# zkMIPS/zkm

Hardware: AMD Instinct MI355X
Metric: segment_proofs_per_sec (higher is better)
Workload: dtype u64 (Goldilocks p = 2^64 - 2^32 + 1, integer modular)

## Files before the change

include/zkm_hip.h:

```cpp
#ifndef ZKM_HIP_H
#define ZKM_HIP_H
#include <stddef.h>
#include <stdint.h>
#ifdef __cplusplus
extern "C" {
#endif

typedef struct zkm_ctx zkm_ctx;
typedef struct zkm_batch zkm_batch;

int zkm_ctx_create(int device, zkm_ctx** out, char** err);
void zkm_ctx_destroy(zkm_ctx* ctx);
int zkm_ctx_synchronize(zkm_ctx* ctx, char** err);
uint64_t zkm_ctx_host_waits(const zkm_ctx* ctx);
void* zkm_ctx_stream(zkm_ctx* ctx);
void zkm_ctx_memory(const zkm_ctx* ctx, size_t* live_bytes, size_t* cached_bytes);
size_t zkm_ctx_resident_bytes(const zkm_ctx* ctx);
void zkm_ctx_trim(zkm_ctx* ctx);
int zkm_ctx_set_tuning(zkm_ctx* ctx, const char* key, uint64_t value, char** err);
int zkm_host_alloc(zkm_ctx* ctx, size_t bytes, void** out, char** err);
int zkm_host_free(zkm_ctx* ctx, void* p);
int zkm_host_register(zkm_ctx* ctx, void* p, size_t bytes, char** err);
int zkm_host_unregister(zkm_ctx* ctx, void* p);
int zkm_dev_alloc(zkm_ctx* ctx, size_t bytes, void** out, char** err);
// ... 30 lines not shown
#define ZKM_POSEIDON_PROBE_PERMUTE_LANE_MFMA 1
#define ZKM_POSEIDON_PROBE_PERMUTE_QUAD 2
#define ZKM_POSEIDON_PROBE_PERMUTE_WIDE 3
#define ZKM_POSEIDON_PROBE_MDS_VALU 4
#define ZKM_POSEIDON_PROBE_MDS_MFMA 5
#define ZKM_POSEIDON_PROBE_MDS_QUAD 6
#define ZKM_POSEIDON_PROBE_MDS_ROWS 7
#define ZKM_POSEIDON_PROBE_GROUP3 8
#define ZKM_POSEIDON_PROBE_GROUP3_QUAD 9
#define ZKM_POSEIDON_PROBE_GROUP2 10
#define ZKM_POSEIDON_PROBE_FOLD 11
#define ZKM_POSEIDON_PROBE_FOLD_TY 12
#define ZKM_POSEIDON_PROBE_SBOX7 13
#define ZKM_POSEIDON_PROBE_SBOX_DELTA 14
#define ZKM_POSEIDON_PROBE_ADD_RC0 15
int zkm_poseidon_selftest(zkm_ctx* ctx, uint32_t probe, uint32_t arg, const uint64_t* in, size_t n, uint64_t* out, char** err);

int zkm_consumer_selftest(zkm_ctx* ctx, const uint64_t* alphas, size_t nalphas, const uint64_t* terms, size_t K, size_t n, uint32_t run,
                          uint64_t* out, char** err);

#define ZKM_POSEIDON_COLS 262
int zkm_poseidon_trace(zkm_ctx* ctx, uint64_t seed, size_t num_perms, unsigned log_n, uint64_t* out_dev, char** err);

int zkm_poseidon_trace_inputs(zkm_ctx* ctx, const uint64_t* inputs, const uint64_t* timestamps, size_t num_perms, unsigned log_n,
                              uint64_t* out_dev, char** err);

#define ZKM_POSEIDON_SPONGE_COLS 110
int zkm_poseidon_sponge_trace(zkm_ctx* ctx, const uint8_t* inputs, const uint64_t* input_off, const uint64_t* meta, size_t nops,
                              unsigned log_n, uint64_t* out_dev, size_t* rows_used_out, char** err);

// ... 483 lines not shown
```

integration/rust/zkm_hip_sys.rs:

```rust
#![allow(non_camel_case_types)]
use std::os::raw::{c_char, c_double, c_int, c_uint, c_void};

#[repr(C)] pub struct zkm_ctx { _p: [u8; 0] }
#[repr(C)] pub struct zkm_batch { _p: [u8; 0] }
#[repr(C)] pub struct zkm_pool { _p: [u8; 0] }
#[repr(C)] pub struct zkm_staged { _p: [u8; 0] }
pub enum zkm_staged_ops {}

#[repr(C)] #[derive(Clone, Copy, Debug, Default)]
pub struct zkm_challenger { pub state: [u64; 12], pub in_buf: [u64; 8], pub out_buf: [u64; 8], pub n_in: u32, pub n_out: u32 }

#[repr(C)] #[derive(Clone, Copy, Debug)]
pub struct zkm_stark_config { pub rate_bits: c_uint, pub cap_height: c_uint, pub pow_bits: c_uint, pub num_challenges: c_uint,
                              pub num_queries: c_uint, pub arity_bits: c_uint, pub final_poly_bits: c_uint }

#[repr(C)] #[derive(Clone, Copy, Debug, Default)]
pub struct zkm_proof_layout {
    pub degree_bits: u64, pub trace_cols: u64, pub aux_cols: u64, pub quotient_polys: u64, pub ctl_zs: u64, pub cap_height: u64,
    pub fri_layers: u64, pub final_poly_len: u64, pub num_queries: u64, pub rate_bits: u64, pub arity_bits: u64,
    pub total_words: usize, pub init_challenger_state: usize, pub trace_cap: usize, pub aux_cap: usize, pub quotient_cap: usize,
    pub local_values: usize, pub next_values: usize, pub aux_polys: usize, pub aux_polys_next: usize, pub ctl_zs_first: usize,
    pub quotient_polys_open: usize, pub commit_phase_merkle_caps: usize, pub final_poly: usize, pub pow_witness: usize,
    pub query_round_proofs: usize, pub query_round_words: usize,
}
// ... 114 lines not shown
pub const ZKM_INSN_LUI: u32 = 0; pub const ZKM_INSN_MUL: u32 = 1; pub const ZKM_INSN_MULT: u32 = 2; pub const ZKM_INSN_MULTU: u32 = 3;
pub const ZKM_INSN_DIV: u32 = 4; pub const ZKM_INSN_DIVU: u32 = 5; pub const ZKM_INSN_MFHI: u32 = 6; pub const ZKM_INSN_MTHI: u32 = 7;
pub const ZKM_INSN_MFLO: u32 = 8; pub const ZKM_INSN_MTLO: u32 = 9; pub const ZKM_INSN_SDC1: u32 = 10; pub const ZKM_INSN_SYNC: u32 = 11;
pub const ZKM_INSN_PREF: u32 = 12;
pub const ZKM_VERIFY_OK: u32 = 0; pub const ZKM_VERIFY_SHAPE: u32 = 1; pub const ZKM_VERIFY_TRANSCRIPT_STATE: u32 = 2;
pub const ZKM_VERIFY_CTL_CHALLENGES: u32 = 3; pub const ZKM_VERIFY_QUOTIENT: u32 = 4; pub const ZKM_VERIFY_POW: u32 = 5;
pub const ZKM_VERIFY_INITIAL_MERKLE: u32 = 6; pub const ZKM_VERIFY_FRI_EVAL: u32 = 7; pub const ZKM_VERIFY_FRI_MERKLE: u32 = 8;
pub const ZKM_VERIFY_FINAL_POLY: u32 = 9; pub const ZKM_VERIFY_CTL_SUM: u32 = 10; pub const ZKM_VERIFY_FAILED: u32 = 11;

pub const ZKM_POSEIDON_OUT_ALL: u32 = 0; pub const ZKM_POSEIDON_OUT_CAPACITY: u32 = 1; pub const ZKM_POSEIDON_OUT_DIGEST: u32 = 2;
pub const ZKM_POSEIDON_PROBE_PERMUTE_LANE: u32 = 0; pub const ZKM_POSEIDON_PROBE_PERMUTE_LANE_MFMA: u32 = 1; pub const ZKM_POSEIDON_PROBE_PERMUTE_QUAD: u32 = 2;
pub const ZKM_POSEIDON_PROBE_PERMUTE_WIDE: u32 = 3; pub const ZKM_POSEIDON_PROBE_MDS_VALU: u32 = 4; pub const ZKM_POSEIDON_PROBE_MDS_MFMA: u32 = 5;
pub const ZKM_POSEIDON_PROBE_MDS_QUAD: u32 = 6; pub const ZKM_POSEIDON_PROBE_MDS_ROWS: u32 = 7; pub const ZKM_POSEIDON_PROBE_GROUP3: u32 = 8;
pub const ZKM_POSEIDON_PROBE_GROUP3_QUAD: u32 = 9; pub const ZKM_POSEIDON_PROBE_GROUP2: u32 = 10; pub const ZKM_POSEIDON_PROBE_FOLD: u32 = 11;
pub const ZKM_POSEIDON_PROBE_FOLD_TY: u32 = 12; pub const ZKM_POSEIDON_PROBE_SBOX7: u32 = 13; pub const ZKM_POSEIDON_PROBE_SBOX_DELTA: u32 = 14;
pub const ZKM_POSEIDON_PROBE_ADD_RC0: u32 = 15;
pub const ZKM_TABLE_POSEIDON: c_int = 0; pub const ZKM_TABLE_LOGIC: c_int = 1; pub const ZKM_TABLE_KECCAK_SPONGE: c_int = 2;
pub const ZKM_TABLE_KECCAK: c_int = 3; pub const ZKM_TABLE_MEMORY: c_int = 4; pub const ZKM_TABLE_POSEIDON_SPONGE: c_int = 5;
pub const ZKM_TABLE_SHA_EXTEND: c_int = 6; pub const ZKM_TABLE_SHA_EXTEND_SPONGE: c_int = 7; pub const ZKM_TABLE_SHA_COMPRESS: c_int = 8;
pub const ZKM_TABLE_SHA_COMPRESS_SPONGE: c_int = 9; pub const ZKM_TABLE_ARITHMETIC: c_int = 10; pub const ZKM_TABLE_CPU: c_int = 11;
pub const ZKM_MEMORY_COLS: usize = 13;
pub const ZKM_ARITHMETIC_COLS: usize = 54;

#[link(name = "zkmhip")]
extern "C" {
    pub fn zkm_ctx_create(device: c_int, out: *mut *mut zkm_ctx, err: *mut *mut c_char) -> c_int;
    pub fn zkm_ctx_destroy(ctx: *mut zkm_ctx);
    pub fn zkm_ctx_synchronize(ctx: *mut zkm_ctx, err: *mut *mut c_char) -> c_int;
    pub fn zkm_ctx_stream(ctx: *mut zkm_ctx) -> *mut c_void;
    pub fn zkm_ctx_memory(ctx: *const zkm_ctx, live_bytes: *mut usize, cached_bytes: *mut usize);
    pub fn zkm_ctx_resident_bytes(ctx: *const zkm_ctx) -> usize;
// ... 288 lines not shown
```

zkm_amd/__init__.py:

```python
import ctypes as C
import os
import re
import subprocess
import weakref

import numpy as np

_HERE = os.path.dirname(os.path.abspath(__file__))
_CSRC = os.path.join(_HERE, "csrc")
_LIB_PATH = os.environ.get("ZKM_HIP_LIB") or os.path.join(_CSRC, "libzkmhip.so")

P = 0xFFFFFFFF00000001


class ZkmError(RuntimeError):
    pass


from . import abi

_H = abi.constants("ZKM_")
POSEIDON_COLS, KECCAK_SPONGE_COLS, LOGIC_COLS, MEMORY_COLS, ARITHMETIC_COLS, KECCAK_COLS, POSEIDON_SPONGE_COLS = (
    _H[n + "_COLS"] for n in ("POSEIDON", "KECCAK_SPONGE", "LOGIC", "MEMORY", "ARITHMETIC", "KECCAK", "POSEIDON_SPONGE"))
TABLE_POSEIDON, TABLE_LOGIC, TABLE_KECCAK_SPONGE, TABLE_KECCAK, TABLE_MEMORY, TABLE_POSEIDON_SPONGE = 0, 1, 2, 3, 4, 5
# ... 923 lines not shown
    def ntt(self, cols, ncols, log_n, inverse=False, coset_shift=0):
        err = C.c_char_p()
        _check(self.L.zkm_ntt(self.h, _data_ptr(cols), ncols, log_n, int(inverse), coset_shift, C.byref(err)), err)
        return cols

    def field_selftest(self, a, b):
        a, b = np.ascontiguousarray(a, dtype=np.uint64), np.ascontiguousarray(b, dtype=np.uint64)
        out = np.zeros(7 * a.size, dtype=np.uint64)
        err = C.c_char_p()
        _check(self.L.zkm_field_selftest(self.h, a.ctypes.data_as(u64p), b.ctypes.data_as(u64p), a.size, out.ctypes.data_as(u64p), C.byref(err)), err)
        return out.reshape(7, -1)

    def poseidon_selftest(self, probe, arg, words):
        probe = POSEIDON_PROBE[probe] if isinstance(probe, str) else int(probe)
        words = np.ascontiguousarray(words, dtype=np.uint64).reshape(-1)
        pairs = probe in (POSEIDON_PROBE["FOLD"], POSEIDON_PROBE["FOLD_TY"])
        per = 2 if pairs else 12
        if words.size % per:
            raise ValueError("poseidon_selftest: %d words are not a whole number of %s" % (words.size, "pairs" if pairs else "states"))
        n = words.size // per
        out = np.zeros(n if pairs else 12 * n, dtype=np.uint64)
        err = C.c_char_p()
        _check(self.L.zkm_poseidon_selftest(self.h, probe, int(arg), words.ctypes.data_as(u64p), n, out.ctypes.data_as(u64p), C.byref(err)), err)
        return out if pairs else out.reshape(-1, 12)

    def consumer_selftest(self, alphas, terms, run=8):
        alphas = np.ascontiguousarray(alphas, dtype=np.uint64).reshape(-1)
        terms = np.ascontiguousarray(terms, dtype=np.uint64)
        if terms.ndim != 2:
            raise ValueError("consumer_selftest: terms must be a (K, n) array")
        K, n = terms.shape
        out = np.zeros(alphas.size * n, dtype=np.uint64)
        err = C.c_char_p()
        _check(self.L.zkm_consumer_selftest(self.h, alphas.ctypes.data_as(u64p), alphas.size, terms.ctypes.data_as(u64p), K, n, int(run),
# ... 1158 lines not shown
```

zkm_amd/csrc/hash.hip:

```cpp
#include <atomic>
#include "poseidon_dev.h"
#include "poseidon_lat_dev.h"
#include "poseidon_mfma_dev.h"
#include "hash_constants_dev.h"
#include "zkm_internal.h"

#ifndef ZKM_LEAF_MFMA_WAVES
#define ZKM_LEAF_MFMA_WAVES (ZKM_MFMA_PARK ? 5 : 4)
#endif

#ifndef ZKM_LATENCY_PRIO
#define ZKM_LATENCY_PRIO 3
#endif
#define ZKM_RAISE_PRIO()                                              \
    do {                                                              \
        if (ZKM_LATENCY_PRIO) __builtin_amdgcn_s_setprio(ZKM_LATENCY_PRIO); \
    } while (0)

__global__ __launch_bounds__(256) void k_poseidon_permute(gl_t* states, size_t k) {
    size_t i = (size_t)blockIdx.x * blockDim.x + threadIdx.x;
    if (i >= k) return;
    uint64_t s[12];
#pragma unroll
    for (int j = 0; j < 12; j++) s[j] = states[i * 12 + j];
// ... 200 lines not shown
                f.template load<true>(s, src, c, nw);
                sponge_lane_valu().permute(s, POSEIDON_OUT_ALL);
            }
        }
    }
    if constexpr (CHUNK) {
        if (!last) {
            f.store_state(s, state, n);
            return;
        }
    }
    f.store_digest(s, digests, f.item, f.live);
}

#define ZKM_LEAF_MFMA_ATTR __attribute__((amdgpu_waves_per_eu(ZKM_LEAF_MFMA_WAVES, ZKM_LEAF_MFMA_WAVES)))

__global__ __launch_bounds__(256) void k_merkle_leaves(const gl_t* __restrict__ lde, size_t nrows, size_t ncols, size_t col_stride,
                                                       gl_t* __restrict__ digests, size_t lde_seg, size_t dig_seg) {
    merkle_leaves_body<sponge_lane_valu>(leaf_cols{lde, ncols, col_stride, lde_seg}, nrows, digests, dig_seg);
}
__global__ __launch_bounds__(256) ZKM_LEAF_MFMA_ATTR void k_merkle_leaves_mfma(const gl_t* __restrict__ lde, size_t nrows, size_t ncols, size_t col_stride,
                                                                              gl_t* __restrict__ digests, size_t lde_seg, size_t dig_seg) {
    merkle_leaves_body<sponge_lane_mfma>(leaf_cols{lde, ncols, col_stride, lde_seg}, nrows, digests, dig_seg);
}
__global__ __launch_bounds__(256) void k_merkle_leaves_quad(const gl_t* __restrict__ lde, size_t nrows, size_t ncols, size_t col_stride,
                                                            gl_t* __restrict__ digests, size_t lde_seg, size_t dig_seg) {
    ZKM_RAISE_PRIO();
    merkle_leaves_body<sponge_quad>(leaf_cols{lde, ncols, col_stride, lde_seg}, nrows, digests, dig_seg);
}
__global__ __launch_bounds__(256) void k_merkle_leaves_wide(const gl_t* __restrict__ lde, size_t nrows, size_t ncols, size_t col_stride,
                                                            gl_t* __restrict__ digests, size_t lde_seg, size_t dig_seg) {
    ZKM_RAISE_PRIO();
    merkle_leaves_body<sponge_wide>(leaf_cols{lde, ncols, col_stride, lde_seg}, nrows, digests, dig_seg);
}

__global__ __launch_bounds__(256) void k_merkle_leaves_chunk(const gl_t* __restrict__ lde, size_t nrows, size_t nc, size_t col_stride,
                                                             gl_t* __restrict__ state, int first, int last, gl_t* __restrict__ digests) {
    merkle_leaves_body<sponge_lane_valu, leaf_cols, true>(leaf_cols{lde, nc, col_stride, 0}, nrows, digests, 0, state, first, last);
}
__global__ __launch_bounds__(256) ZKM_LEAF_MFMA_ATTR void k_merkle_leaves_chunk_mfma(const gl_t* __restrict__ lde, size_t nrows, size_t nc, size_t col_stride,
                                                                                    gl_t* __restrict__ state, int first, int last, gl_t* __restrict__ digests) {
    merkle_leaves_body<sponge_lane_mfma, leaf_cols, true>(leaf_cols{lde, nc, col_stride, 0}, nrows, digests, 0, state, first, last);
}

__global__ __launch_bounds__(256) void k_merkle_leaves_ext(const gl_t* __restrict__ c0, const gl_t* __restrict__ c1,
                                                           size_t nleaves, unsigned arity, gl_t* __restrict__ digests, size_t val_seg, size_t dig_seg) {
    merkle_leaves_body<sponge_lane_valu>(leaf_f2{c0, c1, arity, val_seg}, nleaves, digests, dig_seg);
}
__global__ __launch_bounds__(256) ZKM_LEAF_MFMA_ATTR void k_merkle_leaves_ext_mfma(const gl_t* __restrict__ c0, const gl_t* __restrict__ c1, size_t nleaves,
                                                                                  unsigned arity, gl_t* __restrict__ digests, size_t val_seg, size_t dig_seg) {
    merkle_leaves_body<sponge_lane_mfma>(leaf_f2{c0, c1, arity, val_seg}, nleaves, digests, dig_seg);
}
__global__ __launch_bounds__(256) void k_merkle_leaves_ext_quad(const gl_t* __restrict__ c0, const gl_t* __restrict__ c1, size_t nleaves,
                                                                unsigned arity, gl_t* __restrict__ digests, size_t val_seg, size_t dig_seg) {
    ZKM_RAISE_PRIO();
    merkle_leaves_body<sponge_quad>(leaf_f2{c0, c1, arity, val_seg}, nleaves, digests, dig_seg);
}
__global__ __launch_bounds__(256) void k_merkle_leaves_ext_wide(const gl_t* __restrict__ c0, const gl_t* __restrict__ c1, size_t nleaves,
                                                                unsigned arity, gl_t* __restrict__ digests, size_t val_seg, size_t dig_seg) {
    ZKM_RAISE_PRIO();
// ... 36 lines not shown
    if (nseg == 0 || nseg > 65535) throw std::runtime_error("merkle_leaves_ext: bad segment count");
    zkm_prof_scope ps(c, "merkle_leaves_ext");
    static constexpr decltype(&k_merkle_leaves_ext) kernel[] = {k_merkle_leaves_ext, k_merkle_leaves_ext_mfma, k_merkle_leaves_ext_quad, k_merkle_leaves_ext_wide};
    const merkle_form f = merkle_pick_form(c, nleaves * nseg, true);
    hipLaunchKernelGGL(kernel[f], leaf_grid(f, nleaves, nseg), dim3(256), 0, c->stream, c0, c1, nleaves, arity, digests, val_seg, dig_seg);
    ZKM_HIP_CHECK(hipGetLastError());
}

struct merkle_fused_args {
    const gl_t* children;
    gl_t* parents[3];
    uint32_t levels;
    size_t dig_seg;
};

__global__ __launch_bounds__(256) void k_merkle_fused(merkle_fused_args p) {
    __shared__ uint64_t sh[2][4][256];
    const unsigned tid = threadIdx.x;
    uint64_t s[12];
    {
        const ulonglong2* ch = reinterpret_cast<const ulonglong2*>(p.children + (size_t)blockIdx.z * p.dig_seg + 8 * ((size_t)blockIdx.x * 256 + tid));
        ulonglong2 a = ch[0], b = ch[1], cc = ch[2], d = ch[3];
        s[0] = a.x; s[1] = a.y; s[2] = b.x; s[3] = b.y; s[4] = cc.x; s[5] = cc.y; s[6] = d.x; s[7] = d.y;
    }
#pragma unroll 1
    for (unsigned lvl = 0; lvl < p.levels; lvl++) {
        const unsigned width = 256u >> lvl;
        if (lvl) {
#pragma unroll
            for (int w = 0; w < 4; w++) {
                s[w] = sh[(lvl - 1) & 1][w][2 * tid];
// ... 260 lines not shown
}

void zkm_launch_keccakf(zkm_ctx* c, uint64_t* states, size_t k) {
    if (!k) return;
    zkm_prof_scope ps(c, "keccakf");
    hipLaunchKernelGGL(k_keccakf, dim3((k + 255) / 256), dim3(256), 0, c->stream, states, k);
    ZKM_HIP_CHECK(hipGetLastError());
}

enum {
    PROBE_PERMUTE_LANE = ZKM_POSEIDON_PROBE_PERMUTE_LANE, PROBE_PERMUTE_LANE_MFMA = ZKM_POSEIDON_PROBE_PERMUTE_LANE_MFMA,
    PROBE_PERMUTE_QUAD = ZKM_POSEIDON_PROBE_PERMUTE_QUAD, PROBE_PERMUTE_WIDE = ZKM_POSEIDON_PROBE_PERMUTE_WIDE,
    PROBE_MDS_VALU = ZKM_POSEIDON_PROBE_MDS_VALU, PROBE_MDS_MFMA = ZKM_POSEIDON_PROBE_MDS_MFMA, PROBE_MDS_QUAD = ZKM_POSEIDON_PROBE_MDS_QUAD,
    PROBE_MDS_ROWS = ZKM_POSEIDON_PROBE_MDS_ROWS, PROBE_GROUP3 = ZKM_POSEIDON_PROBE_GROUP3, PROBE_GROUP3_QUAD = ZKM_POSEIDON_PROBE_GROUP3_QUAD,
    PROBE_GROUP2 = ZKM_POSEIDON_PROBE_GROUP2, PROBE_FOLD = ZKM_POSEIDON_PROBE_FOLD, PROBE_FOLD_TY = ZKM_POSEIDON_PROBE_FOLD_TY,
    PROBE_SBOX7 = ZKM_POSEIDON_PROBE_SBOX7, PROBE_SBOX_DELTA = ZKM_POSEIDON_PROBE_SBOX_DELTA, PROBE_ADD_RC0 = ZKM_POSEIDON_PROBE_ADD_RC0
};
static_assert(POSEIDON_OUT_ALL == ZKM_POSEIDON_OUT_ALL && POSEIDON_OUT_CAPACITY == ZKM_POSEIDON_OUT_CAPACITY && POSEIDON_OUT_DIGEST == ZKM_POSEIDON_OUT_DIGEST,
              "include/zkm_hip.h names the output modes of poseidon_dev.h");

template <class Form, int PROBE>
__device__ __forceinline__ void poseidon_probe_lane_body(const uint64_t* __restrict__ in, size_t n, uint64_t* __restrict__ out, unsigned arg) {
    Form f;
    if (!f.take(n)) return;
    typename Form::state_t s;
#pragma unroll
    for (int i = 0; i < 12; i++) s[i] = in[f.item * 12 + i];
    if constexpr (PROBE == PROBE_PERMUTE_LANE || PROBE == PROBE_PERMUTE_LANE_MFMA) {
        f.permute(s, (int)arg);
    } else if constexpr (PROBE == PROBE_MDS_VALU || PROBE == PROBE_MDS_MFMA) {
        f.mds.layer(s, (int)arg);
    } else if constexpr (PROBE == PROBE_MDS_ROWS) {
        if (arg == 0) poseidon_mds_add<false, 0, 4>(s, nullptr);
        else poseidon_mds_add<false, 8, 12>(s, nullptr);
    } else if constexpr (PROBE == PROBE_GROUP3) {
        poseidon_partial_group<3>(s, PC::ZKM_POSEIDON_FUSED_C1[arg], PC::ZKM_POSEIDON_FUSED_C2[arg], PC::ZKM_POSEIDON_FUSED_C3[arg]);
    } else {
        static_assert(PROBE == PROBE_GROUP2, "not a one-lane probe");
        poseidon_partial_group<2>(s, PC::ZKM_POSEIDON_FUSED_C1[7], 0, PC::ZKM_POSEIDON_FUSED_C3[7]);
    }
    if (!f.live) return;
#pragma unroll
    for (int i = 0; i < 12; i++) out[f.item * 12 + i] = s[i];
}
template <int PROBE>
__global__ __launch_bounds__(256) void k_poseidon_probe_lane(const uint64_t* __restrict__ in, size_t n, uint64_t* __restrict__ out, unsigned arg) {
    poseidon_probe_lane_body<sponge_lane_valu, PROBE>(in, n, out, arg);
}
template <int PROBE>
__global__ __launch_bounds__(256) ZKM_LEAF_MFMA_ATTR void k_poseidon_probe_lane_mfma(const uint64_t* __restrict__ in, size_t n, uint64_t* __restrict__ out, unsigned arg) {
    poseidon_probe_lane_body<sponge_lane_mfma, PROBE>(in, n, out, arg);
// ... 24 lines not shown
    sponge_wide f;
    f.take(n);
    const size_t item = f.live ? f.item : n - 1;
    sponge_wide::state_t s;
    s[0] = f.idx < 12 ? in[item * 12 + f.idx] : 0;
    f.permute(s, (int)arg);
    if (f.live && f.idx < 12) out[item * 12 + f.idx] = s[0];
}

template <int PROBE>
__global__ __launch_bounds__(256) void k_poseidon_probe_words(const uint64_t* __restrict__ in, size_t n, uint64_t* __restrict__ out) {
    const size_t i = (size_t)blockIdx.x * blockDim.x + threadIdx.x;
    if (i >= n) return;
    if constexpr (PROBE == PROBE_FOLD) {
        out[i] = poseidon_fold(in[2 * i], in[2 * i + 1]);
    } else if constexpr (PROBE == PROBE_FOLD_TY) {
#if defined(__HIP_DEVICE_COMPILE__)
        out[i] = poseidon_fold_ty(in[2 * i], (uint32_t)in[2 * i + 1]);
#endif
    } else {
        const uint64_t* rc0 = PC::ZKM_POSEIDON_RC;
#pragma unroll
        for (int w = 0; w < 12; w++) {
            const uint64_t x = in[i * 12 + w];
            out[i * 12 + w] = PROBE == PROBE_SBOX7 ? poseidon_sbox7(x) : PROBE == PROBE_SBOX_DELTA ? poseidon_sbox_delta(x) : gl_add_lc(x, rc0[w]);
        }
    }
}

extern "C" int zkm_poseidon_selftest(zkm_ctx* c, uint32_t probe, uint32_t arg, const uint64_t* in, size_t n, uint64_t* out, char** err) {
// ... 4 lines not shown
        bool arg_ok = arg == 0;
        const bool is_out = arg == POSEIDON_OUT_ALL || arg == POSEIDON_OUT_CAPACITY || arg == POSEIDON_OUT_DIGEST;
        const bool is_next = arg == 1 || arg == 2 || arg == 3 || arg == 27 || arg == 28 || arg == 29 || arg == 30;
        switch (probe) {
            case PROBE_PERMUTE_LANE: kernel = k_poseidon_probe_lane<PROBE_PERMUTE_LANE>; arg_ok = is_out; break;
            case PROBE_PERMUTE_LANE_MFMA: kernel = k_poseidon_probe_lane_mfma<PROBE_PERMUTE_LANE_MFMA>; arg_ok = is_out; break;
            case PROBE_PERMUTE_QUAD: kernel = k_poseidon_probe_quad<PROBE_PERMUTE_QUAD>; arg_ok = is_out; lanes = 4; break;
            case PROBE_PERMUTE_WIDE: kernel = k_poseidon_probe_wide; arg_ok = is_out; lanes = 16; break;
            case PROBE_MDS_VALU: kernel = k_poseidon_probe_lane<PROBE_MDS_VALU>; arg_ok = is_next; break;
            case PROBE_MDS_MFMA: kernel = k_poseidon_probe_lane_mfma<PROBE_MDS_MFMA>; arg_ok = is_next; break;
            case PROBE_MDS_QUAD: kernel = k_poseidon_probe_quad<PROBE_MDS_QUAD>; arg_ok = is_next; lanes = 4; break;
            case PROBE_MDS_ROWS: kernel = k_poseidon_probe_lane<PROBE_MDS_ROWS>; arg_ok = arg <= 1; break;
            case PROBE_GROUP3: kernel = k_poseidon_probe_lane<PROBE_GROUP3>; arg_ok = arg < 7; break;
            case PROBE_GROUP3_QUAD: kernel = k_poseidon_probe_quad<PROBE_GROUP3_QUAD>; arg_ok = arg < 7; lanes = 4; break;
            case PROBE_GROUP2: kernel = k_poseidon_probe_lane<PROBE_GROUP2>; break;
            case PROBE_FOLD: case PROBE_FOLD_TY: case PROBE_SBOX7: case PROBE_SBOX_DELTA: case PROBE_ADD_RC0: break;
            default: throw std::runtime_error("zkm_poseidon_selftest: unknown probe");
        }
        if (!arg_ok) throw std::runtime_error("zkm_poseidon_selftest: bad arg for this probe");
        if (!in || !out) throw std::runtime_error("zkm_poseidon_selftest: null argument");
        if (n == 0 || n > ((size_t)1 << 20)) throw std::runtime_error("zkm_poseidon_selftest: n must be 1 .. 2^20");
        const bool pairs = probe == PROBE_FOLD || probe == PROBE_FOLD_TY;
        const size_t in_words = pairs ? 2 * n : 12 * n, out_words = pairs ? n : 12 * n;
        zkm_scratch din(c, in_words * 8), dout(c, out_words * 8);
        ZKM_HIP_CHECK(hipMemcpyAsync(din.p, in, in_words * 8, hipMemcpyHostToDevice, c->stream));
        ZKM_HIP_CHECK(hipMemsetAsync(dout.p, 0, out_words * 8, c->stream));
        const dim3 grid((unsigned)((n * lanes + 255) / 256)), block(256);
        if (kernel) {
            hipLaunchKernelGGL(kernel, grid, block, 0, c->stream, din.as<uint64_t>(), n, dout.as<uint64_t>(), arg);
        } else {
            void (*words)(const uint64_t*, size_t, uint64_t*) =
                probe == PROBE_FOLD ? k_poseidon_probe_words<PROBE_FOLD> : probe == PROBE_FOLD_TY ? k_poseidon_probe_words<PROBE_FOLD_TY> :
                probe == PROBE_SBOX7 ? k_poseidon_probe_words<PROBE_SBOX7> : probe == PROBE_SBOX_DELTA ? k_poseidon_probe_words<PROBE_SBOX_DELTA> :
                                                                                                        k_poseidon_probe_words<PROBE_ADD_RC0>;
            hipLaunchKernelGGL(words, grid, block, 0, c->stream, din.as<uint64_t>(), n, dout.as<uint64_t>());
        }
        ZKM_HIP_CHECK(hipGetLastError());
        ZKM_HIP_CHECK(hipMemcpyAsync(out, dout.p, out_words * 8, hipMemcpyDeviceToHost, c->stream));
        c->sync();
    });
}
```

zkm_amd/csrc/poseidon_dev.h:

```cpp
#pragma once
#include "gl_dev.h"

#undef ZKM_CONSTEXPR
#define ZKM_CONSTEXPR static constexpr
namespace pc_host {
#undef ZKM_CONST
#define ZKM_CONST static const
#include "poseidon_constants.inc"
ZKM_CONST uint64_t ZKM_POSEIDON_ZERO12[12] = {0, 0, 0, 0, 0, 0, 0, 0, 0, 0, 0, 0};
}
#if defined(__HIPCC__)
namespace pc_dev {
#undef ZKM_CONST
#define ZKM_CONST static __device__ __constant__ const
#include "poseidon_constants.inc"
ZKM_CONST uint64_t ZKM_POSEIDON_ZERO12[12] = {0, 0, 0, 0, 0, 0, 0, 0, 0, 0, 0, 0};
}
#endif
#undef ZKM_CONST
#undef ZKM_CONSTEXPR

#if defined(__HIP_DEVICE_COMPILE__)
#define PC pc_dev
#define POSEIDON_SCHED_FENCE() __builtin_amdgcn_sched_barrier(0)
#define POSEIDON_REGION(name) asm volatile("; ZKM_REGION " name)
#else
#define PC pc_host
#define POSEIDON_SCHED_FENCE() ((void)0)
#define POSEIDON_REGION(name) ((void)0)
#endif
// ... 15 lines not shown

GL_HD uint64_t poseidon_fold(uint64_t al, uint64_t ah) {
#if defined(__HIP_DEVICE_COMPILE__)
    const uint64_t t = (uint64_t)(uint32_t)(ah >> 32) * 0xFFFFFFFFu + al;
    uint32_t rhi, wrap;
    uint64_t carry;
    asm("v_add_co_u32_e64 %0, %1, %3, %4\n\ts_nop 1\n\tv_cndmask_b32 %2, 0, -1, %1"
        : "=&v"(rhi), "=&s"(carry), "=v"(wrap)
        : "v"((uint32_t)(t >> 32)), "v"((uint32_t)ah));
    return (((uint64_t)rhi << 32) | (uint32_t)t) + wrap;
#endif
    uint64_t s1 = (uint64_t)(uint32_t)(ah >> 32) * 0xFFFFFFFFu + al;
    uint64_t hs = (uint64_t)(uint32_t)ah + (s1 >> 32);
    uint64_t base = (hs << 32) | (uint32_t)s1;
    return (uint64_t)(uint32_t)(hs >> 32) * 0xFFFFFFFFu + base;
}

template <bool ADD, int ROW0 = 0, int ROW1 = 12>
GL_HD void poseidon_mds_add(uint64_t s[12], const uint64_t* add) {
    uint32_t lo[12], hi[12];
#pragma unroll
    for (int i = 0; i < 12; i++) {
        lo[i] = (uint32_t)s[i];
        hi[i] = (uint32_t)(s[i] >> 32);
    }
    uint32_t C[12] = {17, 15, 41, 16, 2, 28, 13, 13, 39, 18, 34, 20}, diag = 8;
#pragma unroll
    for (int i = 0; i < 12; i++) POSEIDON_OPAQUE(C[i]);
    POSEIDON_OPAQUE(diag);
#pragma unroll
// ... 44 lines not shown
        } else {
            al = gl_mad_imm_sc<poseidon_m1(I, 0)>(d1l, (uint64_t)(uint32_t)c3[I]);
            ah = gl_mad_imm_sc<poseidon_m1(I, 0)>(d1h, c3[I] >> 32);
#pragma unroll
            for (int j = 0; j < 12; j++) {
                al = gl_mad_s(lo[j], PC::ZKM_POSEIDON_M2[I][j], al);
                ah = gl_mad_s(hi[j], PC::ZKM_POSEIDON_M2[I][j], ah);
            }
        }
        s[I] = poseidon_fold(al, ah);
        if ((I & 1) == 1) POSEIDON_SCHED_FENCE();
        poseidon_group_rows<T, I + 1>(s, lo, hi, d1l, d1h, d2l, d2h, c3);
    }
}

template <int T, bool ROW0_ASM = true, class DELTA>
GL_HD void poseidon_partial_group_t(uint64_t s[12], uint64_t c1, uint64_t c2, const uint64_t* c3, DELTA&& delta) {
    uint32_t lo[12], hi[12];
#pragma unroll
    for (int i = 0; i < 12; i++) {
        lo[i] = (uint32_t)s[i];
        hi[i] = (uint32_t)(s[i] >> 32);
    }
    uint64_t al = gl_mad_imm_sc<poseidon_m1(0, 0)>(lo[0], (uint64_t)(uint32_t)c1), ah = gl_mad_imm_sc<poseidon_m1(0, 0)>(hi[0], c1 >> 32);
    if constexpr (ROW0_ASM) {
        poseidon_m_row0<1>(lo, hi, al, ah);
    } else {
#pragma unroll
        for (int j = 1; j < 12; j++) {
            al += (uint64_t)lo[j] * poseidon_m1(0, j);
            ah += (uint64_t)hi[j] * poseidon_m1(0, j);
        }
    }
    const uint64_t d1 = delta(0, poseidon_fold(al, ah));
    const uint32_t d1l = (uint32_t)d1, d1h = (uint32_t)(d1 >> 32);
    uint32_t d2l = 0, d2h = 0;
    POSEIDON_SCHED_FENCE();
    if (T == 3) {
        al = gl_mad_imm_sc<poseidon_m1(0, 0)>(d1l, (uint64_t)(uint32_t)c2);
        ah = gl_mad_imm_sc<poseidon_m1(0, 0)>(d1h, c2 >> 32);
#pragma unroll
        for (int j = 0; j < 12; j++) {
            al = gl_mad_s(lo[j], PC::ZKM_POSEIDON_M2[0][j], al);
            ah = gl_mad_s(hi[j], PC::ZKM_POSEIDON_M2[0][j], ah);
        }
        const uint64_t d2 = delta(1, poseidon_fold(al, ah));
        d2l = (uint32_t)d2;
        d2h = (uint32_t)(d2 >> 32);
        POSEIDON_SCHED_FENCE();
    }
    poseidon_group_rows<T, 0>(s, lo, hi, d1l, d1h, d2l, d2h, c3);
}
template <int T>
GL_HD void poseidon_partial_group(uint64_t s[12], uint64_t c1, uint64_t c2, const uint64_t* c3) {
    poseidon_partial_group_t<T>(s, c1, c2, c3, [](int, uint64_t a) { return poseidon_sbox_delta(a); });
}

enum { POSEIDON_OUT_ALL = 0, POSEIDON_OUT_CAPACITY = 1, POSEIDON_OUT_DIGEST = 2 };

struct poseidon_mds_valu {
    GL_HD void layer(uint64_t s[12], int next) const {
        poseidon_mds_add<true>(s, next < 30 ? &PC::ZKM_POSEIDON_RC[next * 12] : PC::ZKM_POSEIDON_ZERO12);
    }
};

template <class MDS>
// ... 2 lines not shown
    const uint64_t* rc0 = PC::ZKM_POSEIDON_RC;
    POSEIDON_OPAQUE_PTR(rc0);
#pragma unroll
    for (int i = 0; i < 12; i++) s[i] = gl_add_lc(s[i], rc0[i]);
#pragma unroll 1
    for (int r = 0; r < 8; r++) {
        POSEIDON_REGION("full_sbox");
#pragma unroll
        for (int i = 0; i < 12; i++) {
            s[i] = poseidon_sbox7(s[i]);
            if ((i & 1) == 1) POSEIDON_SCHED_FENCE();
        }
        if (r == 3) {
            POSEIDON_REGION("partial_head");
#pragma unroll 1
            for (int g = 0; g < 7; g++) {
                POSEIDON_REGION("partial_group");
                poseidon_partial_group<3>(s, PC::ZKM_POSEIDON_FUSED_C1[g], PC::ZKM_POSEIDON_FUSED_C2[g], PC::ZKM_POSEIDON_FUSED_C3[g]);
                s[0] = poseidon_sbox7(s[0]);
            }
            POSEIDON_REGION("partial_tail");
            const uint64_t* fc1 = PC::ZKM_POSEIDON_FUSED_C1;
            const uint64_t* fc3 = PC::ZKM_POSEIDON_FUSED_C3[7];
            POSEIDON_OPAQUE_PTR(fc1);
            POSEIDON_OPAQUE_PTR(fc3);
            poseidon_partial_group<2>(s, fc1[7], 0, fc3);
        } else if (r == 7 && out != POSEIDON_OUT_ALL) {
            POSEIDON_REGION("last_mds_rows");
            if (out == POSEIDON_OUT_CAPACITY) poseidon_mds_add<false, 8, 12>(s, nullptr);
            else poseidon_mds_add<false, 0, 4>(s, nullptr);
        } else {
            POSEIDON_REGION("full_mds");
            const int next = (r < 3 ? r : 22 + r) + 1;
            mds.layer(s, next);
        }
    }
    POSEIDON_REGION("exit");
    if (out == POSEIDON_OUT_ALL) {
#pragma unroll
        for (int i = 0; i < 12; i++) s[i] = gl_canon(s[i]);
    } else if (out == POSEIDON_OUT_DIGEST) {
// ... 9 lines not shown
```

Before: 17.97.

## Fuse Poseidon partial rounds into groups of four with wide-carry fold

Regroups the 22 partial rounds from seven 3-layer groups plus a 2-layer tail into five 4-layer groups plus a 3-layer tail. It uses precomputed M^4 rows and M/M^2/M^3 first columns, and carries the overflow of the final multiply-add out through a scalar carry mask that a cold path in a new wide fold handles. The aim is fewer fold and row passes per permutation in Merkle hashing. It also pins waves-per-EU on the lane-VALU leaf and fused Merkle kernels, which may change register allocation and spilling.

```diff
diff --git a/include/zkm_hip.h b/include/zkm_hip.h
--- a/include/zkm_hip.h
+++ b/include/zkm_hip.h
@@ -68,6 +68,8 @@
 #define ZKM_POSEIDON_PROBE_SBOX7 13
 #define ZKM_POSEIDON_PROBE_SBOX_DELTA 14
 #define ZKM_POSEIDON_PROBE_ADD_RC0 15
+#define ZKM_POSEIDON_PROBE_GROUP4 17
+#define ZKM_POSEIDON_PROBE_FOLD_WIDE 18
 int zkm_poseidon_selftest(zkm_ctx* ctx, uint32_t probe, uint32_t arg, const uint64_t* in, size_t n, uint64_t* out, char** err);
 
 int zkm_consumer_selftest(zkm_ctx* ctx, const uint64_t* alphas, size_t nalphas, const uint64_t* terms, size_t K, size_t n, uint32_t run,
diff --git a/integration/rust/zkm_hip_sys.rs b/integration/rust/zkm_hip_sys.rs
--- a/integration/rust/zkm_hip_sys.rs
+++ b/integration/rust/zkm_hip_sys.rs
@@ -152,7 +152,7 @@
 pub const ZKM_POSEIDON_PROBE_MDS_QUAD: u32 = 6; pub const ZKM_POSEIDON_PROBE_MDS_ROWS: u32 = 7; pub const ZKM_POSEIDON_PROBE_GROUP3: u32 = 8;
 pub const ZKM_POSEIDON_PROBE_GROUP3_QUAD: u32 = 9; pub const ZKM_POSEIDON_PROBE_GROUP2: u32 = 10; pub const ZKM_POSEIDON_PROBE_FOLD: u32 = 11;
 pub const ZKM_POSEIDON_PROBE_FOLD_TY: u32 = 12; pub const ZKM_POSEIDON_PROBE_SBOX7: u32 = 13; pub const ZKM_POSEIDON_PROBE_SBOX_DELTA: u32 = 14;
-pub const ZKM_POSEIDON_PROBE_ADD_RC0: u32 = 15;
+pub const ZKM_POSEIDON_PROBE_ADD_RC0: u32 = 15; pub const ZKM_POSEIDON_PROBE_GROUP4: u32 = 17; pub const ZKM_POSEIDON_PROBE_FOLD_WIDE: u32 = 18;
 pub const ZKM_TABLE_POSEIDON: c_int = 0; pub const ZKM_TABLE_LOGIC: c_int = 1; pub const ZKM_TABLE_KECCAK_SPONGE: c_int = 2;
 pub const ZKM_TABLE_KECCAK: c_int = 3; pub const ZKM_TABLE_MEMORY: c_int = 4; pub const ZKM_TABLE_POSEIDON_SPONGE: c_int = 5;
 pub const ZKM_TABLE_SHA_EXTEND: c_int = 6; pub const ZKM_TABLE_SHA_EXTEND_SPONGE: c_int = 7; pub const ZKM_TABLE_SHA_COMPRESS: c_int = 8;
diff --git a/zkm_amd/__init__.py b/zkm_amd/__init__.py
--- a/zkm_amd/__init__.py
+++ b/zkm_amd/__init__.py
@@ -961,10 +961,11 @@
     def poseidon_selftest(self, probe, arg, words):
         probe = POSEIDON_PROBE[probe] if isinstance(probe, str) else int(probe)
         words = np.ascontiguousarray(words, dtype=np.uint64).reshape(-1)
-        pairs = probe in (POSEIDON_PROBE["FOLD"], POSEIDON_PROBE["FOLD_TY"])
-        per = 2 if pairs else 12
+        triples = probe == POSEIDON_PROBE["FOLD_WIDE"]
+        pairs = triples or probe in (POSEIDON_PROBE["FOLD"], POSEIDON_PROBE["FOLD_TY"])
+        per = 3 if triples else 2 if pairs else 12
         if words.size % per:
-            raise ValueError("poseidon_selftest: %d words are not a whole number of %s" % (words.size, "pairs" if pairs else "states"))
+            raise ValueError("poseidon_selftest: %d words are not a whole number of %s" % (words.size, "triples" if triples else "pairs" if pairs else "states"))
         n = words.size // per
         out = np.zeros(n if pairs else 12 * n, dtype=np.uint64)
         err = C.c_char_p()
diff --git a/zkm_amd/csrc/hash.hip b/zkm_amd/csrc/hash.hip
--- a/zkm_amd/csrc/hash.hip
+++ b/zkm_amd/csrc/hash.hip
@@ -238,8 +238,9 @@
 }
 
 #define ZKM_LEAF_MFMA_ATTR __attribute__((amdgpu_waves_per_eu(ZKM_LEAF_MFMA_WAVES, ZKM_LEAF_MFMA_WAVES)))
-
-__global__ __launch_bounds__(256) void k_merkle_leaves(const gl_t* __restrict__ lde, size_t nrows, size_t ncols, size_t col_stride,
+#define ZKM_LANE_WAVES_ATTR(n) __attribute__((amdgpu_waves_per_eu(n, n)))
+
+__global__ __launch_bounds__(256) ZKM_LANE_WAVES_ATTR(5) void k_merkle_leaves(const gl_t* __restrict__ lde, size_t nrows, size_t ncols, size_t col_stride,
                                                        gl_t* __restrict__ digests, size_t lde_seg, size_t dig_seg) {
     merkle_leaves_body<sponge_lane_valu>(leaf_cols{lde, ncols, col_stride, lde_seg}, nrows, digests, dig_seg);
 }
@@ -267,7 +268,7 @@
     merkle_leaves_body<sponge_lane_mfma, leaf_cols, true>(leaf_cols{lde, nc, col_stride, 0}, nrows, digests, 0, state, first, last);
 }
 
-__global__ __launch_bounds__(256) void k_merkle_leaves_ext(const gl_t* __restrict__ c0, const gl_t* __restrict__ c1,
+__global__ __launch_bounds__(256) ZKM_LANE_WAVES_ATTR(5) void k_merkle_leaves_ext(const gl_t* __restrict__ c0, const gl_t* __restrict__ c1,
                                                            size_t nleaves, unsigned arity, gl_t* __restrict__ digests, size_t val_seg, size_t dig_seg) {
     merkle_leaves_body<sponge_lane_valu>(leaf_f2{c0, c1, arity, val_seg}, nleaves, digests, dig_seg);
 }
@@ -334,7 +335,7 @@
     size_t dig_seg;
 };
 
-__global__ __launch_bounds__(256) void k_merkle_fused(merkle_fused_args p) {
+__global__ __launch_bounds__(256) ZKM_LANE_WAVES_ATTR(6) void k_merkle_fused(merkle_fused_args p) {
     __shared__ uint64_t sh[2][4][256];
     const unsigned tid = threadIdx.x;
     uint64_t s[12];
@@ -625,7 +626,8 @@
     PROBE_MDS_VALU = ZKM_POSEIDON_PROBE_MDS_VALU, PROBE_MDS_MFMA = ZKM_POSEIDON_PROBE_MDS_MFMA, PROBE_MDS_QUAD = ZKM_POSEIDON_PROBE_MDS_QUAD,
     PROBE_MDS_ROWS = ZKM_POSEIDON_PROBE_MDS_ROWS, PROBE_GROUP3 = ZKM_POSEIDON_PROBE_GROUP3, PROBE_GROUP3_QUAD = ZKM_POSEIDON_PROBE_GROUP3_QUAD,
     PROBE_GROUP2 = ZKM_POSEIDON_PROBE_GROUP2, PROBE_FOLD = ZKM_POSEIDON_PROBE_FOLD, PROBE_FOLD_TY = ZKM_POSEIDON_PROBE_FOLD_TY,
-    PROBE_SBOX7 = ZKM_POSEIDON_PROBE_SBOX7, PROBE_SBOX_DELTA = ZKM_POSEIDON_PROBE_SBOX_DELTA, PROBE_ADD_RC0 = ZKM_POSEIDON_PROBE_ADD_RC0
+    PROBE_SBOX7 = ZKM_POSEIDON_PROBE_SBOX7, PROBE_SBOX_DELTA = ZKM_POSEIDON_PROBE_SBOX_DELTA, PROBE_ADD_RC0 = ZKM_POSEIDON_PROBE_ADD_RC0,
+    PROBE_GROUP4 = ZKM_POSEIDON_PROBE_GROUP4, PROBE_FOLD_WIDE = ZKM_POSEIDON_PROBE_FOLD_WIDE
 };
 static_assert(POSEIDON_OUT_ALL == ZKM_POSEIDON_OUT_ALL && POSEIDON_OUT_CAPACITY == ZKM_POSEIDON_OUT_CAPACITY && POSEIDON_OUT_DIGEST == ZKM_POSEIDON_OUT_DIGEST,
               "include/zkm_hip.h names the output modes of poseidon_dev.h");
@@ -646,6 +648,8 @@
         else poseidon_mds_add<false, 8, 12>(s, nullptr);
     } else if constexpr (PROBE == PROBE_GROUP3) {
         poseidon_partial_group<3>(s, PC::ZKM_POSEIDON_FUSED_C1[arg], PC::ZKM_POSEIDON_FUSED_C2[arg], PC::ZKM_POSEIDON_FUSED_C3[arg]);
+    } else if constexpr (PROBE == PROBE_GROUP4) {
+        poseidon_partial_group4(s, PC::ZKM_POSEIDON_G4_C1[arg], PC::ZKM_POSEIDON_G4_C2[arg], &PC::ZKM_POSEIDON_G4_C3[arg], PC::ZKM_POSEIDON_G4_C4[arg]);
     } else {
         static_assert(PROBE == PROBE_GROUP2, "not a one-lane probe");
         poseidon_partial_group<2>(s, PC::ZKM_POSEIDON_FUSED_C1[7], 0, PC::ZKM_POSEIDON_FUSED_C3[7]);
@@ -700,6 +704,14 @@
     if (i >= n) return;
     if constexpr (PROBE == PROBE_FOLD) {
         out[i] = poseidon_fold(in[2 * i], in[2 * i + 1]);
+    } else if constexpr (PROBE == PROBE_FOLD_WIDE) {
+        const uint64_t carries = in[3 * i + 2];
+#if defined(__HIP_DEVICE_COMPILE__)
+        const uint64_t cl = __ballot((int)(carries & 1)), ch = __ballot((int)((carries >> 1) & 1));
+#else
+        const uint64_t cl = carries & 1, ch = (carries >> 1) & 1;
+#endif
+        out[i] = poseidon_fold_wide(in[3 * i], in[3 * i + 1], cl, ch);
     } else if constexpr (PROBE == PROBE_FOLD_TY) {
 #if defined(__HIP_DEVICE_COMPILE__)
         out[i] = poseidon_fold_ty(in[2 * i], (uint32_t)in[2 * i + 1]);
@@ -734,14 +746,15 @@
             case PROBE_GROUP3: kernel = k_poseidon_probe_lane<PROBE_GROUP3>; arg_ok = arg < 7; break;
             case PROBE_GROUP3_QUAD: kernel = k_poseidon_probe_quad<PROBE_GROUP3_QUAD>; arg_ok = arg < 7; lanes = 4; break;
             case PROBE_GROUP2: kernel = k_poseidon_probe_lane<PROBE_GROUP2>; break;
-            case PROBE_FOLD: case PROBE_FOLD_TY: case PROBE_SBOX7: case PROBE_SBOX_DELTA: case PROBE_ADD_RC0: break;
+            case PROBE_GROUP4: kernel = k_poseidon_probe_lane<PROBE_GROUP4>; arg_ok = arg < 5; break;
+            case PROBE_FOLD_WIDE: case PROBE_FOLD: case PROBE_FOLD_TY: case PROBE_SBOX7: case PROBE_SBOX_DELTA: case PROBE_ADD_RC0: break;
             default: throw std::runtime_error("zkm_poseidon_selftest: unknown probe");
         }
         if (!arg_ok) throw std::runtime_error("zkm_poseidon_selftest: bad arg for this probe");
         if (!in || !out) throw std::runtime_error("zkm_poseidon_selftest: null argument");
         if (n == 0 || n > ((size_t)1 << 20)) throw std::runtime_error("zkm_poseidon_selftest: n must be 1 .. 2^20");
-        const bool pairs = probe == PROBE_FOLD || probe == PROBE_FOLD_TY;
-        const size_t in_words = pairs ? 2 * n : 12 * n, out_words = pairs ? n : 12 * n;
+        const bool pairs = probe == PROBE_FOLD || probe == PROBE_FOLD_TY, triples = probe == PROBE_FOLD_WIDE;
+        const size_t in_words = triples ? 3 * n : pairs ? 2 * n : 12 * n, out_words = pairs || triples ? n : 12 * n;
         zkm_scratch din(c, in_words * 8), dout(c, out_words * 8);
         ZKM_HIP_CHECK(hipMemcpyAsync(din.p, in, in_words * 8, hipMemcpyHostToDevice, c->stream));
         ZKM_HIP_CHECK(hipMemsetAsync(dout.p, 0, out_words * 8, c->stream));
@@ -751,6 +764,7 @@
         } else {
             void (*words)(const uint64_t*, size_t, uint64_t*) =
                 probe == PROBE_FOLD ? k_poseidon_probe_words<PROBE_FOLD> : probe == PROBE_FOLD_TY ? k_poseidon_probe_words<PROBE_FOLD_TY> :
+                probe == PROBE_FOLD_WIDE ? k_poseidon_probe_words<PROBE_FOLD_WIDE> :
                 probe == PROBE_SBOX7 ? k_poseidon_probe_words<PROBE_SBOX7> : probe == PROBE_SBOX_DELTA ? k_poseidon_probe_words<PROBE_SBOX_DELTA> :
                                                                                                         k_poseidon_probe_words<PROBE_ADD_RC0>;
             hipLaunchKernelGGL(words, grid, block, 0, c->stream, din.as<uint64_t>(), n, dout.as<uint64_t>());
diff --git a/zkm_amd/csrc/poseidon_dev.h b/zkm_amd/csrc/poseidon_dev.h
--- a/zkm_amd/csrc/poseidon_dev.h
+++ b/zkm_amd/csrc/poseidon_dev.h
@@ -7,6 +7,7 @@
 #undef ZKM_CONST
 #define ZKM_CONST static const
 #include "poseidon_constants.inc"
+#include "poseidon_group4.inc"
 ZKM_CONST uint64_t ZKM_POSEIDON_ZERO12[12] = {0, 0, 0, 0, 0, 0, 0, 0, 0, 0, 0, 0};
 }
 #if defined(__HIPCC__)
@@ -14,6 +15,7 @@
 #undef ZKM_CONST
 #define ZKM_CONST static __device__ __constant__ const
 #include "poseidon_constants.inc"
+#include "poseidon_group4.inc"
 ZKM_CONST uint64_t ZKM_POSEIDON_ZERO12[12] = {0, 0, 0, 0, 0, 0, 0, 0, 0, 0, 0, 0};
 }
 #endif
@@ -59,6 +61,53 @@
     uint64_t hs = (uint64_t)(uint32_t)ah + (s1 >> 32);
     uint64_t base = (hs << 32) | (uint32_t)s1;
     return (uint64_t)(uint32_t)(hs >> 32) * 0xFFFFFFFFu + base;
+}
+
+GL_HD uint64_t gl_mad_s_co(uint32_t x, uint32_t m, uint64_t c, uint64_t& carry) {
+#if defined(__HIP_DEVICE_COMPILE__)
+    uint64_t r;
+    asm("v_mad_u64_u32 %0, %1, %2, %3, %4" : "=v"(r), "=s"(carry) : "v"(x), "s"(m), "v"(c));
+    return r;
+#else
+    const uint64_t r = (uint64_t)x * m + c;
+    carry = r < c;
+    return r;
+#endif
+}
+
+GL_HD uint64_t poseidon_fold_wide(uint64_t al, uint64_t ah, uint64_t cl, uint64_t ch) {
+    uint64_t r;
+#if defined(__HIP_DEVICE_COMPILE__)
+    uint64_t t;
+    uint32_t e, rlo, rhi;
+    asm("v_mad_u64_u32 %0, vcc, %2, -1, %3\n\tv_cndmask_b32 %1, 0, -1, vcc" : "=&v"(t), "=&v"(e) : "v"((uint32_t)(ah >> 32)), "v"(al) : "vcc");
+    asm("v_add_co_u32 %0, vcc, %3, %2\n\t"
+        "v_addc_co_u32 %1, vcc, 0, %4, vcc\n\t"
+        "v_add_co_u32 %1, vcc, %1, %5\n\t"
+        "v_cndmask_b32 %2, 0, -1, vcc\n\t"
+        "v_add_co_u32 %0, vcc, %0, %2\n\t"
+        "v_addc_co_u32 %1, vcc, 0, %1, vcc"
+        : "=&v"(rlo), "=&v"(rhi), "+&v"(e)
+        : "v"((uint32_t)t), "v"((uint32_t)(t >> 32)), "v"((uint32_t)ah)
+        : "vcc");
+    r = ((uint64_t)rhi << 32) | rlo;
+    if (__builtin_expect((cl | ch) != 0, 0)) {
+        asm volatile("; ZKM_COLD");
+        const unsigned lane = __lane_id() & 63;
+        if ((cl >> lane) & 1) r = gl_add_lc(r, GL_EPS);
+        if ((ch >> lane) & 1) r = r ? r - 1 : GL_P - 1;
+    }
+#else
+    const uint64_t p1 = (uint64_t)(uint32_t)(ah >> 32) * 0xFFFFFFFFu;
+    uint64_t t = p1 + al;
+    if (t < al) t += GL_EPS;
+    const uint64_t hs = (t >> 32) + (uint32_t)ah;
+    r = (hs << 32) | (uint32_t)t;
+    if (hs >> 32) r += GL_EPS;
+    if (cl) r = gl_add_lc(r, GL_EPS);
+    if (ch) r = r ? r - 1 : GL_P - 1;
+#endif
+    return r;
 }
 
 template <bool ADD, int ROW0 = 0, int ROW1 = 12>
@@ -133,8 +182,34 @@
     }
 }
 
+template <int I>
+GL_HD void poseidon_group4_rows(uint64_t s[12], const uint32_t lo[12], const uint32_t hi[12], uint32_t d1l, uint32_t d1h, uint32_t d2l, uint32_t d2h,
+                                uint32_t d3l, uint32_t d3h, const uint64_t* c4) {
+    if constexpr (I < 12) {
+        static_assert(PC::ZKM_POSEIDON_G4_DCOL[0][I] == poseidon_m1(I, 0) && PC::ZKM_POSEIDON_G4_DCOL[1][I] == PC::ZKM_POSEIDON_M2[I][0] &&
+                      PC::ZKM_POSEIDON_G4_DCOL[2][I] == PC::ZKM_POSEIDON_M3[I][0], "first columns of M, M^2, M^3");
+        uint64_t al = gl_mad_imm_sc<poseidon_m1(I, 0)>(d3l, (uint64_t)(uint32_t)c4[I]), ah = gl_mad_imm_sc<poseidon_m1(I, 0)>(d3h, c4[I] >> 32);
+        al = gl_mad_s(d2l, PC::ZKM_POSEIDON_G4_DCOL[1][I], al);
+        ah = gl_mad_s(d2h, PC::ZKM_POSEIDON_G4_DCOL[1][I], ah);
+        al = gl_mad_s(d1l, PC::ZKM_POSEIDON_G4_DCOL[2][I], al);
+        ah = gl_mad_s(d1h, PC::ZKM_POSEIDON_G4_DCOL[2][I], ah);
+#pragma unroll
+        for (int j = 0; j < 11; j++) {
+            al = gl_mad_s(lo[j], PC::ZKM_POSEIDON_M4[I][j], al);
+            ah = gl_mad_s(hi[j], PC::ZKM_POSEIDON_M4[I][j], ah);
+        }
+        uint64_t cl, ch;
+        al = gl_mad_s_co(lo[11], PC::ZKM_POSEIDON_M4[I][11], al, cl);
+        ah = gl_mad_s_co(hi[11], PC::ZKM_POSEIDON_M4[I][11], ah, ch);
+        s[I] = poseidon_fold_wide(al, ah, cl, ch);
+        if ((I & 1) == 1) POSEIDON_SCHED_FENCE();
+        poseidon_group4_rows<I + 1>(s, lo, hi, d1l, d1h, d2l, d2h, d3l, d3h, c4);
+    }
+}
+
 template <int T, bool ROW0_ASM = true, class DELTA>
-GL_HD void poseidon_partial_group_t(uint64_t s[12], uint64_t c1, uint64_t c2, const uint64_t* c3, DELTA&& delta) {
+GL_HD void poseidon_partial_group_t(uint64_t s[12], uint64_t c1, uint64_t c2, const uint64_t* c3, DELTA&& delta, const uint64_t* c4 = nullptr) {
+    static_assert(T == 2 || T == 3 || T == 4, "groups of two, three or four layers");
     uint32_t lo[12], hi[12];
 #pragma unroll
     for (int i = 0; i < 12; i++) {
@@ -155,7 +230,7 @@
     const uint32_t d1l = (uint32_t)d1, d1h = (uint32_t)(d1 >> 32);
     uint32_t d2l = 0, d2h = 0;
     POSEIDON_SCHED_FENCE();
-    if (T == 3) {
+    if (T >= 3) {
         al = gl_mad_imm_sc<poseidon_m1(0, 0)>(d1l, (uint64_t)(uint32_t)c2);
         ah = gl_mad_imm_sc<poseidon_m1(0, 0)>(d1h, c2 >> 32);
 #pragma unroll
@@ -168,7 +243,23 @@
         d2h = (uint32_t)(d2 >> 32);
         POSEIDON_SCHED_FENCE();
     }
-    poseidon_group_rows<T, 0>(s, lo, hi, d1l, d1h, d2l, d2h, c3);
+    if constexpr (T == 4) {
+        al = gl_mad_s(d1l, PC::ZKM_POSEIDON_M2[0][0], gl_mad_imm_sc<poseidon_m1(0, 0)>(d2l, (uint64_t)(uint32_t)c3[0]));
+        ah = gl_mad_s(d1h, PC::ZKM_POSEIDON_M2[0][0], gl_mad_imm_sc<poseidon_m1(0, 0)>(d2h, c3[0] >> 32));
+#pragma unroll
+        for (int j = 0; j < 12; j++) {
+            al = gl_mad_s(lo[j], PC::ZKM_POSEIDON_M3[0][j], al);
+            ah = gl_mad_s(hi[j], PC::ZKM_POSEIDON_M3[0][j], ah);
+        }
+        const uint64_t d3 = delta(2, poseidon_fold(al, ah));
+        POSEIDON_SCHED_FENCE();
+        poseidon_group4_rows<0>(s, lo, hi, d1l, d1h, d2l, d2h, (uint32_t)d3, (uint32_t)(d3 >> 32), c4);
+    } else {
+        poseidon_group_rows<T, 0>(s, lo, hi, d1l, d1h, d2l, d2h, c3);
+    }
+}
+GL_HD void poseidon_partial_group4(uint64_t s[12], uint64_t c1, uint64_t c2, const uint64_t* c3, const uint64_t* c4) {
+    poseidon_partial_group_t<4>(s, c1, c2, c3, [](int, uint64_t a) { return poseidon_sbox_delta(a); }, c4);
 }
 template <int T>
 GL_HD void poseidon_partial_group(uint64_t s[12], uint64_t c1, uint64_t c2, const uint64_t* c3) {
@@ -201,17 +292,17 @@
         if (r == 3) {
             POSEIDON_REGION("partial_head");
 #pragma unroll 1
-            for (int g = 0; g < 7; g++) {
-                POSEIDON_REGION("partial_group");
-                poseidon_partial_group<3>(s, PC::ZKM_POSEIDON_FUSED_C1[g], PC::ZKM_POSEIDON_FUSED_C2[g], PC::ZKM_POSEIDON_FUSED_C3[g]);
+            for (int g = 0; g < 5; g++) {
+                POSEIDON_REGION("partial_group4");
+                poseidon_partial_group4(s, PC::ZKM_POSEIDON_G4_C1[g], PC::ZKM_POSEIDON_G4_C2[g], &PC::ZKM_POSEIDON_G4_C3[g], PC::ZKM_POSEIDON_G4_C4[g]);
                 s[0] = poseidon_sbox7(s[0]);
             }
             POSEIDON_REGION("partial_tail");
-            const uint64_t* fc1 = PC::ZKM_POSEIDON_FUSED_C1;
-            const uint64_t* fc3 = PC::ZKM_POSEIDON_FUSED_C3[7];
-            POSEIDON_OPAQUE_PTR(fc1);
-            POSEIDON_OPAQUE_PTR(fc3);
-            poseidon_partial_group<2>(s, fc1[7], 0, fc3);
+            const uint64_t* tc12 = PC::ZKM_POSEIDON_G4_TAIL_C12;
+            const uint64_t* tc3 = PC::ZKM_POSEIDON_G4_TAIL_C3;
+            POSEIDON_OPAQUE_PTR(tc12);
+            POSEIDON_OPAQUE_PTR(tc3);
+            poseidon_partial_group<3>(s, tc12[0], tc12[1], tc3);
         } else if (r == 7 && out != POSEIDON_OUT_ALL) {
             POSEIDON_REGION("last_mds_rows");
             if (out == POSEIDON_OUT_CAPACITY) poseidon_mds_add<false, 8, 12>(s, nullptr);
diff --git a/zkm_amd/csrc/poseidon_group4.inc b/zkm_amd/csrc/poseidon_group4.inc
--- /dev/null
+++ b/zkm_amd/csrc/poseidon_group4.inc
@@ -0,0 +1,79 @@
+ZKM_CONSTEXPR uint32_t ZKM_POSEIDON_M4[12][12] = {
+    {381558488u, 369288112u, 374533544u, 369959168u, 369454632u, 373358944u, 370265576u, 368886800u, 375007320u, 369607648u, 370277912u, 373854368u},
+    {373854368u, 357623704u, 358824096u, 362304040u, 357790720u, 359163384u, 361468960u, 358453864u, 358738272u, 362530840u, 358873600u, 358107144u},
+    {370277912u, 363385904u, 359530600u, 358628928u, 362580520u, 359632512u, 359263656u, 362413968u, 360578840u, 358445408u, 364635672u, 358873600u},
+    {369607648u, 357841672u, 363242464u, 357426104u, 357304992u, 362611176u, 357965408u, 358508792u, 362402336u, 358324552u, 358445408u, 362530840u},
+    {375007320u, 358891216u, 359772456u, 363367680u, 358082088u, 359247008u, 363011304u, 359184368u, 360706264u, 362402336u, 360578840u, 358738272u},
+    {368886800u, 362336792u, 358838416u, 357739464u, 361725808u, 357942552u, 357503856u, 362032872u, 359184368u, 358508792u, 362413968u, 358453864u},
+    {370265576u, 357418192u, 363216664u, 357590848u, 357148184u, 362702816u, 357138904u, 357503856u, 363011304u, 357965408u, 359263656u, 361468960u},
+    {373358944u, 358888936u, 358959456u, 362859992u, 357846656u, 358765576u, 362702816u, 357942552u, 359247008u, 362611176u, 359632512u, 359163384u},
+    {369454632u, 360921296u, 359059288u, 357057728u, 361200024u, 357846656u, 357148184u, 361725808u, 358082088u, 357304992u, 362580520u, 357790720u},
+    {369959168u, 358531384u, 362427136u, 358297672u, 357057728u, 362859992u, 357590848u, 357739464u, 363367680u, 357426104u, 358628928u, 362304040u},
+    {374533544u, 359211952u, 360256728u, 362427136u, 359059288u, 358959456u, 363216664u, 358838416u, 359772456u, 363242464u, 359530600u, 358824096u},
+    {369288112u, 362193128u, 359211952u, 358531384u, 360921296u, 358888936u, 357418192u, 362336792u, 358891216u, 357841672u, 363385904u, 357623704u},
+};
+ZKM_CONSTEXPR uint32_t ZKM_POSEIDON_G4_DCOL[3][12] = {
+    {25u, 20u, 34u, 18u, 39u, 13u, 13u, 28u, 2u, 16u, 41u, 15u},
+    {5642u, 5364u, 6818u, 4880u, 5870u, 6080u, 5302u, 5356u, 6238u, 5368u, 4914u, 5952u},
+    {1525684u, 1411808u, 1436396u, 1476584u, 1444108u, 1416584u, 1506604u, 1420320u, 1422580u, 1480072u, 1418228u, 1438872u},
+};
+ZKM_CONST uint64_t ZKM_POSEIDON_G4_C1[5] = {
+    0x3cc3f892184df408ULL, 0x7159cd30c3ac118eULL, 0x15a16a8a8322d458ULL, 0x0c49366bb25e8513ULL,
+    0xe89cd854d5d01d33ULL,
+};
+ZKM_CONST uint64_t ZKM_POSEIDON_G4_C2[5] = {
+    0x5677c8b64ff234acULL, 0x50c17f4e8bc2a7b5ULL, 0x81fc8da6ab2368baULL, 0xa5927abe1e6e71c4ULL,
+    0xfc39f87979d52a85ULL,
+};
+ZKM_CONST uint64_t ZKM_POSEIDON_G4_C3[5] = {
+    0x56363c738e3fbfabULL, 0xd119def35a30b511ULL, 0x13b33fa406f06ba9ULL, 0xaec1adbccd06f9a4ULL,
+    0xbb167cb775013794ULL,
+};
+ZKM_CONST uint64_t ZKM_POSEIDON_G4_C4[5][12] = {
+    {
+        0x4822d44c5c940cdfULL, 0x2cc4aa4032cbf6acULL, 0xe6be7d5a2368895cULL, 0x961baf62fe7fa095ULL,
+        0x7f3edb213dbb1f5cULL, 0x1ac9cf28f9aa1cd3ULL, 0xfea41595b7f73ebfULL, 0xd88c5ce5821f7a63ULL,
+        0xd5ea8555519631caULL, 0x62be3869c9142420ULL, 0x585e5f597f13d523ULL, 0x2bd7a94353a94ffcULL,
+    },
+    {
+        0x436097890c42a26eULL, 0x172a4c9c9ae52c96ULL, 0x07d08f116ef3d9c7ULL, 0x5fde687057199718ULL,
+        0xcf672c8182dd46ebULL, 0xdc58d7161d799053ULL, 0x6bf3f56d5212969bULL, 0x1e007f513a27ed73ULL,
+        0x2ade2297ecf78357ULL, 0xd803bb9b51dfd95aULL, 0x6dc69efd9d6ba243ULL, 0xd887fe85249eab19ULL,
+    },
+    {
+        0x08f4722492add0b6ULL, 0x2f5fd1d28a279fdeULL, 0x07c7f9e981722b7bULL, 0x97505612541c2d5eULL,
+        0x7782663a37a840c5ULL, 0x5e09ffb3682ae462ULL, 0xbbba7f5d71d79e1bULL, 0xf79598b32c274153ULL,
+        0x23288e9e34803b65ULL, 0x46439c4592cd6b33ULL, 0xf78cf4e27ab47e9dULL, 0x7637a0057515aeabULL,
+    },
+    {
+        0xcc150d05db000c2eULL, 0xfcdbe290741ae0a3ULL, 0xea162e05bbb13f9fULL, 0x020f71d621aebcacULL,
+        0xf648ab3364ccc3e4ULL, 0x1c7f8e93fb60b44bULL, 0xf24e256405535ad0ULL, 0x2fc38a416cdad5ddULL,
+        0x77253f38cc60426fULL, 0x424fb3b0ca022740ULL, 0x525d77f29091cd2aULL, 0xa58f127fe9671002ULL,
+    },
+    {
+        0x652aa51d5c9ad32fULL, 0x329003249dbc1524ULL, 0x57f3fcd79d86f429ULL, 0xec3fc43b256e0cd4ULL,
+        0x3344bc0244fb6db5ULL, 0x85c1b417903ca64fULL, 0x1792372a9c826c32ULL, 0x5f8b4341b5a2d69fULL,
+        0x1ceaac904fc12aaaULL, 0x975cf07e5ce9c21eULL, 0x8a0607636e8f2a4eULL, 0x359c54f24b9bd779ULL,
+    },
+};
+ZKM_CONST uint64_t ZKM_POSEIDON_G4_TAIL_C12[2] = {
+    0x4d61e56a525d225aULL, 0xd258ba14008de909ULL,
+};
+ZKM_CONST uint64_t ZKM_POSEIDON_G4_TAIL_C3[12] = {
+    0x375669aaabd2fb2dULL, 0x5d7afc7e16b18675ULL, 0x539fe49fa660144bULL, 0x51e0838410adde7cULL,
+    0x2675e1ec7b25cb8eULL, 0x484b608a7b8c72daULL, 0x431f34928329c035ULL, 0x90180d93cb9c8dffULL,
+    0x65245b014a5b4d6cULL, 0xafb14099820da0f3ULL, 0x1827bb99fce6d88aULL, 0xf2efce47e0b0d461ULL,
+};
+#ifdef __cplusplus
+constexpr bool zkm_poseidon_group4_bounds() {
+    for (int i = 0; i < 12; i++) {
+        uint64_t w = (uint64_t)ZKM_POSEIDON_G4_DCOL[0][i] + ZKM_POSEIDON_G4_DCOL[1][i] + ZKM_POSEIDON_G4_DCOL[2][i];
+        for (int j = 0; j < 12; j++) w += ZKM_POSEIDON_M4[i][j];
+        if (w - ZKM_POSEIDON_M4[i][11] + 1 > (1ULL << 32)) return false;
+        if (w + 1 > (1ULL << 33)) return false;
+    }
+    return true;
+}
+static_assert(sizeof(ZKM_POSEIDON_M4[0][0]) == 4, "(a) an entry of M^4 fits a 32-bit multiplier");
+static_assert(zkm_poseidon_group4_bounds(), "(b), (c): a half-sum of an M^4 row is exact before its last multiply-add and carries at most once");
+#endif
```

Result: faster. 18.29 (median of 6 runs) (+1.8%).
